# TUMFTM/CamRaDepth

Measured on AMD Instinct MI355X. Metric: training images/sec at 256x416 bf16, higher is better.
Workload: dtype bf16; 1 GPU; CamRaDepth base (image+radar) train step, 8x7x256x416 per GPU, bf16 MFMA / fp32 accumulate, diffGradNorm + OneCycleLR, Dropout2d/DropPath on; global_batch=8, parallelism=dp1, hip_graph=True

## Files before the change

### camradepth_amd/csrc/train_ops.hip

```cpp
#include <math.h>
#include "common.h"

namespace {

constexpr int TPB = 256;

constexpr int OPT_CHUNK = 4096;

template <bool GATED, bool CLIP = false>
__global__ __launch_bounds__(TPB) void k_dgn_norm(const float* p, const float* g, const long long* seg_off, const int* blk2seg,
                                                  const int* blk2chunk, float wd, const float* hp, float* norm_sq,
                                                  const unsigned char* active, int* gate, long long ps = 0) {
  if (hp) wd = hp[3];
  const int t = blk2seg[blockIdx.x];
  if (active && !active[t]) {
    if (threadIdx.x == 0) {
      norm_sq[blockIdx.x] = 0.f;
      if (CLIP) norm_sq[blockIdx.x + ps] = norm_sq[blockIdx.x + 2 * ps] = norm_sq[blockIdx.x + 3 * ps] = 0.f;
    }
    return;
  }
  const long long beg = seg_off[2 * t] + (long long)blk2chunk[blockIdx.x] * OPT_CHUNK;
  long long end = beg + OPT_CHUNK;
  if (end > seg_off[2 * t + 1]) end = seg_off[2 * t + 1];
// ... 191 lines not shown
  const long long tid = (long long)blockIdx.x * TPB + threadIdx.x, stride = (long long)gridDim.x * TPB;
  float4* a4 = reinterpret_cast<float4*>(a + head);
  float4* b4 = reinterpret_cast<float4*>(b + head);
  for (long long i = tid; i < nvec; i += stride) {
    const float4 x = a4[i], y = b4[i];
    a4[i] = y; b4[i] = x;
  }
  const long long tail0 = head + 4 * nvec, rem = head + (n - tail0);
  for (long long i = tid; i < rem; i += stride) {
    const long long j = i < head ? i : tail0 + (i - head);
    const float x = a[j], y = b[j];
    a[j] = y; b[j] = x;
  }
}

constexpr int WP_CO = 16, WP_ELEMS = 512;
__global__ __launch_bounds__(TPB) void k_weight_pack(const crd_pack_entry* tab) {
  __shared__ float tile[WP_CO * WP_ELEMS];
  const crd_pack_entry e = tab[blockIdx.y];
  int ci_t = (WP_ELEMS / e.taps) & ~7;
  if (ci_t < 8) ci_t = 8;
  if (ci_t > 64) ci_t = 64;
  const int n_ci = (e.Cin_pad + ci_t - 1) / ci_t, n_co = (e.Cout_pad + WP_CO - 1) / WP_CO;
  const int per_co = ci_t * e.taps;
  for (int tl = blockIdx.x; tl < n_ci * n_co; tl += gridDim.x) {
    const int co0 = (tl / n_ci) * WP_CO, ci0 = (tl % n_ci) * ci_t;
    __syncthreads();
    for (int i = threadIdx.x; i < WP_CO * per_co; i += TPB) {
      const int co = co0 + i / per_co, r = i % per_co;
      const int ci = ci0 + r / e.taps, tap = r % e.taps;
      float v = 0.f;
      if (co < e.Cout && ci < e.Cin_pad) {
        const int cr = e.cmap ? e.cmap[ci] : (ci < e.Cin_ref ? ci : -1);
        if (cr >= 0) v = e.src[((long long)co * e.Cin_ref + cr) * e.taps + tap];
      }
      tile[i] = v;
    }
    __syncthreads();
    if (e.dst_fwd) {
      for (int i = threadIdx.x; i < WP_CO * per_co; i += TPB) {
        const int cl = i % ci_t, r = i / ci_t;
        const int tap = r % e.taps, col = r / e.taps;
        const int co = co0 + col, ci = ci0 + cl;
        if (co < e.Cout && ci < e.Cin_pad) {
          const float v = tile[col * per_co + cl * e.taps + tap];
          const long long o = ((long long)co * e.taps + tap) * e.Cin_pad + ci;
          if (e.dst_f32) reinterpret_cast<float*>(e.dst_fwd)[o] = e.dst_f32 == 2 ? bf_round(v) : v;
          else reinterpret_cast<bf16_t*>(e.dst_fwd)[o] = f2bf(v);
        }
      }
    }
    if (e.dst_dgrad || e.dst_scatter) {
      for (int i = threadIdx.x; i < WP_CO * per_co; i += TPB) {
        const int col = i % WP_CO, r = i / WP_CO;
        const int tap = r % e.taps, cl = r / e.taps;
        const int co = co0 + col, ci = ci0 + cl;
        if (co < e.Cout_pad && ci < e.Cin_pad) {
          const bf16_t q = f2bf(tile[col * per_co + cl * e.taps + tap]);
          if (e.dst_dgrad) {
            if (e.dgrad_ld == 0) reinterpret_cast<bf16_t*>(e.dst_dgrad)[((long long)ci * e.taps + tap) * e.Cout_pad + co] = q;
            else {
              const int rr = ci - e.dgrad_row0;
              if (rr >= 0 && rr < e.dgrad_rows)
                reinterpret_cast<bf16_t*>(e.dst_dgrad)[((long long)rr * e.taps + tap) * e.dgrad_ld + e.dgrad_coff + co] = q;
            }
          }
          if (e.dst_scatter) reinterpret_cast<bf16_t*>(e.dst_scatter)[((long long)tap * e.Cin_pad + ci) * e.Cout_pad + co] = q;
        }
      }
    }
  }
}

__global__ __launch_bounds__(TPB) void k_wgrad_unpack(const crd_unpack_entry* tab, int accumulate) {
  const crd_unpack_entry e = tab[blockIdx.y];
  const long long n = (long long)e.Cout * e.taps * e.Cin_pad;
  for (long long i = (long long)blockIdx.x * TPB + threadIdx.x; i < n; i += (long long)gridDim.x * TPB) {
    const int ci = (int)(i % e.Cin_pad);
    const long long r = i / e.Cin_pad;
    const int tap = (int)(r % e.taps), co = (int)(r / e.taps);
    const int cr = e.cmap ? e.cmap[ci] : (ci < e.Cin_ref ? ci : -1);
    if (cr < 0) continue;
    float* d = e.dst + ((long long)co * e.Cin_ref + cr) * e.taps + tap;
    float v;
    if (e.src_sum) {
      const crd_sum_t* src = reinterpret_cast<const crd_sum_t*>(e.src);
      long long q = src[i], q1 = 0, q2 = 0, q3 = 0;
      int rp = 1;
      for (; rp + 3 <= e.replicas; rp += 3) {
        q1 += src[(long long)rp * e.replica_stride + i];
        q2 += src[(long long)(rp + 1) * e.replica_stride + i];
        q3 += src[(long long)(rp + 2) * e.replica_stride + i];
      }
      for (; rp < e.replicas; ++rp) q += src[(long long)rp * e.replica_stride + i];
      v = (float)(q + q1 + q2 + q3) * (1.f / GRAD_ONE);
    } else {
      const float* src = reinterpret_cast<const float*>(e.src);
      float v1 = 0.f, v2 = 0.f, v3 = 0.f;
      v = src[i];
      int rp = 1;
      for (; rp + 3 <= e.replicas; rp += 3) {
        v1 += src[(long long)rp * e.replica_stride + i];
        v2 += src[(long long)(rp + 1) * e.replica_stride + i];
        v3 += src[(long long)(rp + 2) * e.replica_stride + i];
      }
      for (; rp < e.replicas; ++rp) v += src[(long long)rp * e.replica_stride + i];
      v += (v1 + v2) + v3;
    }
    *d = accumulate ? *d + v : v;
  }
}

__global__ __launch_bounds__(TPB) void k_dropout_masks(float* out, const float* keep, int rows, int cols, unsigned long long seed,
                                                       unsigned long long* counter) {
  const unsigned long long epoch = *counter;
  const long long total = (long long)rows * cols;
  for (long long i = (long long)blockIdx.x * TPB + threadIdx.x; i < total; i += (long long)gridDim.x * TPB) {
    const int r = (int)(i / cols);
    const float kp = keep[r];
    const unsigned long long h = splitmix64(splitmix64(seed ^ (epoch * 0xD1342543DE82EF95ull)) + (unsigned long long)i);
    const float u = (float)(h >> 40) * (1.0f / 16777216.0f);
    out[i] = u < kp ? 1.0f / kp : 0.0f;
  }
}
__global__ void k_counter_inc(unsigned long long* counter) { *counter += 1; }
// ... 99 lines not shown
  hipLaunchKernelGGL(k_swap_f32, dim3(blocks_for(work, TPB, 4096)), dim3(TPB), 0, as_stream(stream), a, b, (long long)n, head, nvec);
  CRD_LAUNCH_CHECK("crd_swap_f32");
  return CRD_OK;
}

extern "C" int crd_dropout_masks(float* out, const float* keep, int32_t rows, int32_t cols, uint64_t seed, uint64_t* counter,
                                 crd_stream_t stream) {
  CRD_CHECK_ARG(out && keep && counter && rows > 0 && cols > 0, "crd_dropout_masks: bad argument");
  hipLaunchKernelGGL(k_dropout_masks, dim3(blocks_for((long long)rows * cols, TPB, 64)), dim3(TPB), 0, as_stream(stream), out, keep, rows,
                     cols, (unsigned long long)seed, reinterpret_cast<unsigned long long*>(counter));
  hipLaunchKernelGGL(k_counter_inc, dim3(1), dim3(1), 0, as_stream(stream), reinterpret_cast<unsigned long long*>(counter));
  CRD_LAUNCH_CHECK("crd_dropout_masks");
  return CRD_OK;
}

extern "C" int crd_weight_pack(const crd_pack_entry* table_dev, int32_t n, int64_t max_elems, crd_stream_t stream) {
  CRD_CHECK_ARG(table_dev && n > 0 && max_elems > 0, "crd_weight_pack: bad argument");
  long long tiles = (max_elems + WP_CO * WP_ELEMS - 1) / (WP_CO * WP_ELEMS) * 2;
  if (tiles < 1) tiles = 1;
  if (tiles > 96) tiles = 96;
  hipLaunchKernelGGL(k_weight_pack, dim3((unsigned)tiles, n), dim3(TPB), 0, as_stream(stream), table_dev);
  CRD_LAUNCH_CHECK("crd_weight_pack");
  return CRD_OK;
}

extern "C" int crd_wgrad_unpack(const crd_unpack_entry* table_dev, int32_t n, int64_t max_elems, int32_t accumulate,
                                crd_stream_t stream) {
  CRD_CHECK_ARG(table_dev && n > 0 && max_elems > 0, "crd_wgrad_unpack: bad argument");
  hipLaunchKernelGGL(k_wgrad_unpack, dim3(blocks_for(max_elems, TPB, 2048), n), dim3(TPB), 0, as_stream(stream), table_dev, accumulate);
  CRD_LAUNCH_CHECK("crd_wgrad_unpack");
  return CRD_OK;
}
```

### camradepth_amd/engine.py

```python
import bisect
import os
from types import SimpleNamespace as Rec

import torch

from . import lib as L
from . import trace
from . import plan_tables as tables
from . import plan_values
from .config import MID_CHANNELS, UNSUP_CLASSES
from .plan_desc import make_desc
from .plan_values import (BF16, F32, SUM, PM, ConvW, Op, _BufPtr, _Lazy, _WPtr, conv3p_tile, dgrad_flops, fp8_tile,
                          fused_reduce_tile_ok, gn_small_tile, gnbwd_tile, gngemm_tile, halo_tile, igemm_tile, nbytes,
                          persistent_conv3, rup, wgrad3_tile, wgrad_tile)

_DEV = os.environ.get("CRD_DEV_SWITCHES") == "1"


def _dev_flag(name):
    return _DEV and os.environ.get(name) is not None


def _dev_int(name, default):
    return int(os.environ.get(name, default)) if _DEV else int(default)
# ... 1 lines not shown

FUSE_GN_RED_MAXPIX = _dev_int("CRD_FUSE_GN_RED_MAXPIX", 416)


def gn_conv_default():
    return _dev_int("CRD_GN_CONV", 2)


MLP_FUSED = _dev_int("CRD_MLP_FUSED", 1) != 0
MLP_FUSED_MAXPIX = _dev_int("CRD_MLP_FUSED_MAXPIX", 128)
FC2_FOLD_MINROWS = _dev_int("CRD_FC2_FOLD_MINROWS", 16384)
GN_CONV_MAXROWS = _dev_int("CRD_GN_CONV_MAXROWS", 1 << 30)
W3_LATE_WGS = _dev_int("CRD_W3_LATE_WGS", 160)
LATE = 3
DW_REPLICAS = tables.DW_REPLICAS
HEAD_ROWS = 64
GNB_FC1 = _dev_int("CRD_GNB_FC1", 7)
GNB_SR = _dev_int("CRD_GNB_SR", 15)
QSR_GROUP = _dev_int("CRD_QSR_GROUP", 4)


class Plan:
    def __init__(self, model, B, H, W, training):
        cfg = model.cfg
        assert H % 32 == 0 and W % 32 == 0, "H and W must be multiples of 32 (SURVEY.md section 8 note on 900x1600)"
        self.model, self.cfg, self.B, self.H, self.W, self.training = model, cfg, B, H, W, training
        self.dev = model.flat.device
        self.lib = L.load()
        self.fwd, self.bwd_groups, self.bwd_tags = [], [], []
        self._tag = "enc0"
# ... 959 lines not shown
        bad = ~torch.isfinite(self.model.flat_grad)
        if not bool(bad.any()) and bool(torch.isfinite(self.zb_arena).all()):
            return
        where = int(bad.nonzero()[0]) if bool(bad.any()) else -1
        pname = "zb_arena"
        for n_, o_ in zip(self.model._names, self.model._offsets):
            if o_ <= where:
                pname = n_
        for k in self.keep:
            if isinstance(k, tuple) and k[0] == "buf" and k[5].is_floating_point() and not bool(torch.isfinite(k[5].float()).all()):
                print("[crd] non-finite buffer", k[1:5], flush=True)
        raise L.CrdError(f"non-finite gradient after op {i} {op.name} (first bad param {pname})")

    def _unpack(self, tag, stream):
        if tag in self.unpack_ranges:
            lo, hi, mx = self.unpack_ranges[tag]
            L.check(self.lib.crd_wgrad_unpack(self.unpack_table.data_ptr() + lo * self.unpack_stride, hi - lo, mx, 1, stream),
                    "crd_wgrad_unpack")

    def pack(self, lo=None, hi=None):
        st = L.stream()
        i0 = 0 if lo is None else bisect.bisect_left(self.pack_offs, lo)
        i1 = self.n_pack if hi is None else bisect.bisect_left(self.pack_offs, hi)
        if i1 > i0:
            L.check(self.lib.crd_weight_pack(self.pack_table.data_ptr() + i0 * self.pack_stride, i1 - i0,
                                             max(self.pack_elems[i0:i1]), st), "crd_weight_pack")
        base = self.model.flat.data_ptr()
        for cw, cin16 in self.fp8_convs:
            off = (self.p(cw.name + ".weight").data_ptr() - base) // 4
            if (lo is None or off >= lo) and (hi is None or off < hi):
                L.check(self.lib.crd_weight_quant_fp8(cw.w_fwd.data_ptr(), cw.cout, 9, cw.cin_pad, cin16, cw.w8.data_ptr(),
                                                      cw.w8_scales.data_ptr(), st), "crd_weight_quant_fp8")
        for cw, Wt, rows, K, W8, W8s in self.fp8_kcat:
            off = (self.p(cw.name + ".weight").data_ptr() - base) // 4
            if (lo is None or off >= lo) and (hi is None or off < hi):
                L.check(self.lib.crd_weight_quant_fp8(Wt.data_ptr(), rows, 9, K, K, W8.data_ptr(), W8s.data_ptr(), st), "crd_weight_quant_fp8")
        if lo is None and hi is None:
            self.packed_version = getattr(self.model, "_param_version", 0)

    def ensure_packed(self):
        if self.packed_version != getattr(self.model, "_param_version", 0):
# ... 43 lines not shown
```

### camradepth_amd/lib.py

```python
import ctypes as C
import os
import struct

import torch

_HERE = os.path.dirname(os.path.abspath(__file__))
LIB_PATH = os.environ.get("CRD_LIB") or os.path.join(_HERE, "libcamradepth_hip.so")


class CrdError(RuntimeError):
    pass


class ConvDesc(C.Structure):
    _fields_ = [
        ("x", C.c_void_p), ("x_ld", C.c_int32), ("x_coff", C.c_int32),
        ("B", C.c_int32), ("IH", C.c_int32), ("IW", C.c_int32), ("Cin", C.c_int32),
        ("w", C.c_void_p), ("Cout", C.c_int32), ("KH", C.c_int32), ("KW", C.c_int32),
        ("stride", C.c_int32), ("pad", C.c_int32), ("OH", C.c_int32), ("OW", C.c_int32),
        ("gather_mode", C.c_int32),
        ("y", C.c_void_p), ("y_ld", C.c_int32), ("y_coff", C.c_int32), ("y_f32", C.c_int32),
        ("out_mode", C.c_int32), ("patch_k", C.c_int32), ("patch_c", C.c_int32),
        ("bias", C.c_void_p), ("bias_bstride", C.c_int32), ("act", C.c_int32),
        ("res", C.c_void_p), ("res_ld", C.c_int32), ("res_scale", C.c_void_p),
# ... 42 lines not shown


class MlpDesc(C.Structure):
    _fields_ = [(n, C.c_void_p) for n in ("x1", "x1_stats", "norm_gamma", "norm_beta", "w_fc1", "b_fc1", "norm1_gamma", "norm1_beta",
                                          "w9", "b_dw", "norm2_gamma", "norm2_beta", "w_fc2", "xn", "h1", "h2", "h3", "h1_stats",
                                          "h2_stats", "fc2_partials")] + \
               [(n, C.c_int32) for n in ("B", "H", "W", "C", "hidden")]


class UnpackEntry(C.Structure):
    _fields_ = [
        ("src", C.c_void_p), ("dst", C.c_void_p), ("cmap", C.c_void_p),
        ("Cout", C.c_int32), ("Cin_ref", C.c_int32), ("taps", C.c_int32), ("Cin_pad", C.c_int32),
        ("replicas", C.c_int32), ("src_sum", C.c_int32), ("replica_stride", C.c_int64),
    ]


class DgnDesc(C.Structure):
    _fields_ = [(n, C.c_void_p) for n in ("p", "g", "exp_avg", "exp_avg_sq", "prev_grad", "exp_grad_norm", "factor", "parts", "seg_off",
                                          "blk2seg", "blk2chunk", "active", "hp_dev", "gate", "clip", "ema")] + \
               [("parts_stride", C.c_int64), ("n_tensors", C.c_int32), ("n_blocks", C.c_int32)] + \
               [(n, C.c_float) for n in ("lr", "beta1", "beta2", "eps", "weight_decay")] + \
               [("step", C.c_int32), ("max_norm", C.c_float), ("ema_decay", C.c_float),
                ("ema_warmup", C.c_int32), ("ema_n", C.c_int32), ("ema_base", C.c_int32)]


_lib = None
ABI_VERSION = 13


# ... 31 lines not shown
    "crd_conv_igemm": "pp", "crd_conv_igemm_route": "ppi", "crd_gn_conv": "ppp", "crd_gn_conv2": "ppppp", "crd_gn_bwd_conv": "ppp", "crd_pw_narrow_supported": "iii", "crd_tune_pw_narrow": "i", "crd_conv3x3_fp8": "ppfp", "crd_amax_bf16": "pliiipp", "crd_quant_fp8": "pliiipiifp",
    "crd_weight_quant_fp8": "piiiippp", "crd_conv3x3_fp8_dgrad": "pppp", "crd_gn_bwd_apply_fp8": "piiipiiiiiipippipppppiipiippp",
    "crd_fp8_scale_update": "ppifip", "crd_quant_fp8_dev": "pliiipiipp", "crd_tune_conv3x3_small_grid": "i", "crd_tune_igemm_reg_epilogue": "i", "crd_conv_wgrad": "pp", "crd_conv_wgrad_splits": "p", "crd_conv_wgrad_route": "ppi", "crd_wgrad_group_build": "piplp", "crd_conv_wgrad_grouped": "ppp",
    "crd_gn_stats": "piiiiiippp", "crd_gn_apply": "piiiiiipippipPiiip".replace("P", "p"),
    "crd_gn_bwd_reduce": "piiipiiiiiipippippplp", "crd_gn_bwd_apply": "piiipiiiiiipippipppppiiiipipp",
    "crd_gn_launch_shape": "iiiippp",
    "crd_dwconv3x3": "piiiippipppippppppp", "crd_dwconv3x3_wgrad": "ppiiiipipippp",
    "crd_attn_scores": "ppiiiiifppp", "crd_attn_scores_fp8": "ppiiiiffppp", "crd_attn_fwd": "ppiiiiifpppppppppp", "crd_attn_xbar": "ppppiiipp", "crd_attn_xbar_proj": "pppppiiippp", "crd_attn_vec_bwd": "ppiiifppp", "crd_attn_out_residual": "pppppiiipp", "crd_attn_out_residual_stats": "pppppiiippp",
    "crd_attn_out_bwd": "ppppiiipppp", "crd_attn_out_bwd_blocks": "iii", "crd_attn_out_bwd_gn": "ppppiiippppppppppp", "crd_attn_scores_bwd": "ppppiiiiifpppp", "crd_attn_bwd": "ppppiiiiifpppppifppp", "crd_attn_scores_bwd_partials": "iiiii", "crd_sum_partials_bf16": "pilplp", "crd_gsum_to_bf16": "pplp",
    "crd_attn_bwd_fused_supported": "iiiii", "crd_attn_bwd_fused": "ppppppp" "iiiii" "f" "ppppp" "ppppppp" "p", "crd_attn_dk_fold": "pilpl" "pp" "iii" "f" "pp" "p",
    "crd_bicubic2x": "piiiiiipiip", "crd_bicubic2x_fp8": "piiiiiipiifpiip", "crd_gn_apply_fp8": "piiiiiipippippiifpiip", "crd_bicubic2x_bwd": "piiiiiipiiip",
    "crd_input_grad": "ppppiiiiiipp",
    "crd_nchw_to_pm": "piiiipiiip", "crd_pm_to_nchw": "piiiiiiipp", "crd_seg_argmax": "piiiiipiiip", "crd_scale_f32": "pplfp",
    "crd_slice_copy": "piipiiliip", "crd_f32_to_bf16_rows": "pipiiliplpiip", "crd_dropout_masks": "ppiiLpp", "crd_sigmoid_bwd": "pplp", "crd_head_conv2_fwd": "pppiiippiip", "crd_head_conv2_bwd": "ppiippiiippip", "crd_head_conv2_bwd_data": "ppiippiiipp", "crd_head_conv2_wgrad": "ppiipiiipip",
    "crd_weight_pack": "pilp", "crd_wgrad_unpack": "pilip",
    "crd_assemble_input": "pppiiifpp", "crd_gt_pyramid": "piiifppppp",
    "crd_augment_draw": "ppiiiiifffffffiLLp", "crd_augment_lut": "piipp", "crd_augment_assemble": "pppppppiiiiifppppp",
    "crd_augment_gather": "ppppiiiiiippppp", "crd_gt_pyramid_from_full": "piiipppp",
    "crd_radar_project": "pppiipppipiiiffpppppppp", "crd_radar_rasterize": "ppppppppiipiiiiiplppp",
    "crd_lidar_project": "pppiippppippipppipiiiffLLpppppppppp", "crd_lidar_ground_truth": "pppppppppiipiiiiipppipLplpppp",
    "crd_depth_unproject": "piiiiipipiiLLLipppppp", "crd_point_cloud": "piiiiipipiiLLLipppipplpppppp",
    "crd_bev_grid": "ppppiiipiLLLiiLLiiiplppppppp",
    "crd_occupancy_update": "pppiiipipipiiiiLiLLLLiiiiiipppppplpppppp",
    "crd_distance_field": "piiiiiippplppppp", "crd_field_paths": "pppiipLpppiiiiiippppppp",
    "crd_nav_field": "piiippipLiiipppp", "crd_nav_paths": "ppiipLppiiipppppp",
    "crd_map_objects": "piiiiiiipLplpppppp",
    "crd_track_objects": "pppp" "iiiii" "LLLL" "ii" "ppppppppp" "p",
    "crd_match_scan": "ppp" "iii" "pipi" "iii" "LLLL" "i" "ppp" "ii" "p" "il" "pl" "ppppppp" "p",
    "crd_plan_rollouts": "pppp" "iiii" "pLpp" "iiii" "ppp" "iii" "LL" "pLL" "iiiii" "pl" "pppp" "ppppp" "p" "p",
    "crd_viz_range": "piiiiipplpp", "crd_viz_draw": "piiiippffipiiffipllp", "crd_seg_labels": "piiiipp",
# ... 44 lines not shown
    if nonfinite(reset=False):
        v = torch.full_like(v, float("nan"))
    return v


def f64_bits(x):
    return struct.unpack("<Q", struct.pack("<d", float(x)))[0]


def check(rc, what=""):
    if rc != 0:
        msg = load().crd_last_error().decode()
        raise CrdError(f"{what} failed with status {rc}: {msg}")


def conv_route(desc):
    buf = C.create_string_buffer(96)
    check(load().crd_conv_igemm_route(C.byref(desc), buf, len(buf)), "crd_conv_igemm_route")
    return buf.value.decode()


def wgrad_route(desc):
    buf = C.create_string_buffer(96)
    check(load().crd_conv_wgrad_route(C.byref(desc), buf, len(buf)), "crd_conv_wgrad_route")
    return buf.value.decode()


def gn_launch_shape(P, Cn, B, kind):
    out = (C.c_int32 * 3)()
    ptr = [C.cast(C.byref(out, 4 * i), C.c_void_p) for i in range(3)]
# ... 11 lines not shown
```

### camradepth_amd/plan_tables.py

```python
import ctypes as C

import torch

from . import lib as L
from .plan_values import BF16, F32, SUM, rup

SEGMENTS = ["dec", "enc3", "enc2", "enc1", "enc0"]
DW_REPLICAS = 16


def _struct_table(entries, dev):
    if not entries:
        return torch.zeros(8, dtype=torch.uint8, device=dev)
    raw = b"".join(bytes(e) for e in entries)
    return torch.frombuffer(bytearray(raw), dtype=torch.uint8).to(dev)


def _pack_entry(plan, name, dims, cmap=None, **dst):
    e = L.PackEntry()
    e.src = plan.p(name + ".weight").data_ptr()
    e.cmap = cmap.data_ptr() if cmap is not None else None
    e.Cout, e.Cin_ref, e.taps, e.Cin_pad, e.Cout_pad = dims
    for k, v in dst.items():
        setattr(e, k, v.data_ptr() if isinstance(v, torch.Tensor) else v)
    return e


def build_pack_table(plan):
    dev = plan.dev
    sizes = lambda cw: (cw.cout * cw.taps * cw.cin_pad, cw.cin_pad * cw.taps * cw.cout_pad)
# ... 18 lines not shown
            cw.cmap_dev = torch.tensor(cw.cmap, dtype=torch.int32, device=dev)
        dst = {k: t for k, t in (("dst_fwd", cw.w_fwd), ("dst_dgrad", cw.w_dgrad), ("dst_scatter", cw.w_scatter)) if t is not None}
        entries.append((_pack_entry(plan, cw.name, cw.dims, cw.cmap_dev, **dst), max(n_fwd, n_bwd)))
    for (cw, Wt, ld, coff, row0, rows) in plan.kcat_entries:
        entries.append((_pack_entry(plan, cw.name, cw.dims, cw.cmap_dev, dst_dgrad=Wt, dgrad_ld=ld, dgrad_coff=coff, dgrad_row0=row0,
                                    dgrad_rows=rows), cw.cin_pad * cw.taps * cw.cout_pad))
    for (name, hid, w9, fmt) in plan.dw_entries:
        entries.append((_pack_entry(plan, name, (1, hid, 9, hid, 8), dst_fwd=w9, dst_f32=fmt), 9 * hid))
    base = plan.model.flat.data_ptr()
    entries.sort(key=lambda en: en[0].src)
    plan.pack_offs = [(e.src - base) // 4 for e, _ in entries]
    plan.pack_elems = [n for _, n in entries]
    plan.pack_table = _struct_table([e for e, _ in entries], dev)
    plan.pack_stride = C.sizeof(L.PackEntry)
    plan.n_pack = len(entries)


def stream3_splits(lib, B, ih, iw, cin, cout, k=3, stride=1, pad=1, wg_budget=0):
    probe = L.WgradDesc()
    probe.B, probe.IH, probe.IW, probe.OH, probe.OW = B, ih, iw, (ih + 2 * pad - k) // stride + 1, (iw + 2 * pad - k) // stride + 1
    probe.Cin, probe.Cout, probe.KH, probe.KW, probe.stride, probe.pad = cin, cout, k, k, stride, pad
    probe.wg_budget = wg_budget
    return int(lib.crd_conv_wgrad_splits(C.byref(probe)))


def place_weight_gradients(plan):
    out = []
    for cw in plan.convs:
        if cw.frozen:
            continue
# ... 38 lines not shown
        items.append((cw.tag, _unpack_entry(dst=plan.g(cw.name + ".weight"), dims=cw.dims[:4], cmap=cw.cmap_dev, **parts), nel))
    for name, hid, dw10, tag in plan.dw_grads:
        for which, taps, row in (("weight", 9, 0), ("bias", 1, 9)):
            items.append((tag, _unpack_entry(dw10.t.data_ptr() + row * hid * 8, plan.g(name + "." + which), (1, hid, taps, hid),
                                             replicas=DW_REPLICAS, replica_stride=10 * hid), taps * hid))
    for name, Cn, rows, R, tag, off, stride in plan.row_grads:
        items.append((tag, _unpack_entry(rows.t.data_ptr() + 8 * off, plan.g(name), (1, Cn, 1, Cn), replicas=R, replica_stride=stride), Cn))
    items.sort(key=lambda it: SEGMENTS.index(it[0]))
    plan.unpack_ranges = {}
    for i, (tag, _, nel) in enumerate(items):
        lo, _, mx = plan.unpack_ranges.get(tag, (i, i, 1))
        plan.unpack_ranges[tag] = (lo, i + 1, max(mx, nel))
    plan.unpack_table = _struct_table([u for _, u, _ in items], plan.dev)
    plan.unpack_stride = C.sizeof(L.UnpackEntry)
    plan.n_unpack, plan.max_unpack = len(items), max([1] + [nel for _, _, nel in items])


def order_backward(plan):
    written = {}
    plan.bwd, plan.bwd_segments = [], []
    for grp, tag in zip(reversed(plan.bwd_groups), reversed(plan.bwd_tags)):
        if plan.bwd_segments and plan.bwd_segments[-1][0] == tag:
            plan.bwd_segments[-1][2] = len(plan.bwd) + len(grp)
        else:
            plan.bwd_segments.append([tag, len(plan.bwd), len(plan.bwd) + len(grp)])
        for op in grp:
            if op.region is not None:
                key, c0, c1 = op.region[:-2], op.region[-2], op.region[-1]
                prev = written.setdefault(key, [])
                overlap = [r for r in prev if r[0] < c1 and c0 < r[1]]
# ... 11 lines not shown
```

### include/camradepth_hip.h

```cpp
#ifndef CAMRADEPTH_HIP_H
#define CAMRADEPTH_HIP_H

#include <stdint.h>

#ifdef __cplusplus
extern "C" {
#endif

typedef void* crd_stream_t;

#define CRD_OK 0
#define CRD_E_INVALID (-1)
#define CRD_E_UNSUPPORTED (-2)
#define CRD_E_LAUNCH (-3)

typedef int64_t crd_sum_t;
#define CRD_STAT_FRAC_BITS 20
#define CRD_GRAD_FRAC_BITS 44
int crd_nonfinite_status(int32_t reset, crd_stream_t stream);
int crd_nonfinite_capture(int32_t* window_flag, crd_stream_t stream);

const char* crd_last_error(void);
#define CRD_ABI_VERSION 13
int crd_version(void);
// ... 235 lines not shown
  int32_t dst_f32;
  int32_t dgrad_ld, dgrad_coff, dgrad_row0, dgrad_rows;
} crd_pack_entry;
int crd_weight_pack(const crd_pack_entry* table_dev, int32_t n, int64_t max_elems, crd_stream_t stream);
typedef struct {
  const void* src;
  float* dst;
  const int32_t* cmap;
  int32_t Cout, Cin_ref, taps, Cin_pad;
  int32_t replicas;
  int32_t src_sum;
  int64_t replica_stride;
} crd_unpack_entry;
int crd_wgrad_unpack(const crd_unpack_entry* table_dev, int32_t n, int64_t max_elems, int32_t accumulate,
                     crd_stream_t stream);

int crd_dropout_masks(float* out, const float* keep, int32_t rows, int32_t cols, uint64_t seed, uint64_t* counter,
                      crd_stream_t stream);

int crd_assemble_input(const void* img_u8, const float* radar, const float* rad_vel, int32_t B, int32_t H, int32_t W,
                       float max_depth, float* out, crd_stream_t stream);
int crd_gt_pyramid(const float* depth, int32_t B, int32_t H, int32_t W, float max_depth, float* full, float* half,
                   float* quarter, float* eighth, crd_stream_t stream);
int crd_resize_nearest_u8(const void* src, int32_t B, int32_t SH, int32_t SW, int32_t C, void* dst, int32_t DH, int32_t DW,
                          crd_stream_t stream);
int crd_resize_labels_nearest(const void* src_u8, int32_t B, int32_t SH, int32_t SW, int32_t rows, int64_t* dst, int32_t DH,
                              int32_t DW, crd_stream_t stream);

#define CRD_AUGMENT_WORDS 8
#define CRD_AUGMENT_STREAM 0xA0761D6478BD642Full
// ... 182 lines not shown
```

Before: 478.2 images/s.

## Tile weight pack/unpack via precomputed work-item lists with larger LDS tiles

Replaces the 2D-grid weight pack and wgrad unpack kernels with tiled versions that use larger shared-memory tiles, padded strides, fast integer division and unrolled gathers. The host precomputes flat work-item lists, so each block handles a balanced tile or a run of small entries instead of launching max_elems-sized grids per entry. The goal is to cut wasted blocks and uncoalesced strided accesses in per-step weight repacking and gradient unpacking. In exchange the host-side planning gets more complex, and the tile-shape heuristics may not suit every layer.

```diff
diff --git a/camradepth_amd/csrc/train_ops.hip b/camradepth_amd/csrc/train_ops.hip
--- a/camradepth_amd/csrc/train_ops.hip
+++ b/camradepth_amd/csrc/train_ops.hip
@@ -229,101 +229,300 @@
   }
 }
 
-constexpr int WP_CO = 16, WP_ELEMS = 512;
-__global__ __launch_bounds__(TPB) void k_weight_pack(const crd_pack_entry* tab) {
-  __shared__ float tile[WP_CO * WP_ELEMS];
+constexpr int WP_LDS = 12288;
+constexpr int UP_LDS = 4608;
+constexpr int PACK_ITEM_WORK = WP_LDS;
+constexpr int UNPACK_ITEM_WORK = UP_LDS;
+constexpr int PACK_MAX_TAPS = 64, UNPACK_MAX_TAPS = 512;
+constexpr int PACK_LOAD_UNR = 16, PACK_UNR = 8, UNPACK_UNR = 4, UNPACK_UNR1 = 8;
+
+struct FastDiv { unsigned m; int one; };
+__host__ __device__ inline FastDiv fast_div(int d) { return FastDiv{d <= 1 ? 0u : 0xFFFFFFFFu / (unsigned)d + 1u, d <= 1 ? 1 : 0}; }
+__device__ __forceinline__ int fdiv(int r, FastDiv f) { return (int)__umulhi((unsigned)r, f.m) + r * f.one; }
+template <typename T>
+__device__ __forceinline__ __attribute__((address_space(1))) T* as_global(T* p) {
+  return (__attribute__((address_space(1))) T*)p;
+}
+__host__ __device__ inline int imin(int a, int b) { return a < b ? a : b; }
+__host__ __device__ inline int imax(int a, int b) { return a > b ? a : b; }
+__host__ __device__ inline int pack_co_ext(const crd_pack_entry& e) { return imax(e.Cout, e.Cout_pad); }
+
+__host__ __device__ inline void pack_shape(const crd_pack_entry& e, int& co_t, int& ci_t) {
+  const int tp = e.taps | 1, cin8 = (e.Cin_pad + 7) & ~7, co_ext = pack_co_ext(e);
+  for (co_t = 64;; co_t >>= 1) {
+    const int per = WP_LDS / imin(co_t, co_ext);
+    ci_t = imin(imin(((per - 1) / tp) & ~7, cin8), 512);
+    if (co_t == 16 || ci_t >= imin(cin8, 16)) break;
+  }
+  if (ci_t < 8) ci_t = 8;
+}
+
+__host__ __device__ inline void unpack_shape(const crd_unpack_entry& e, int& ci_sh, int& rows) {
+  const int tp = e.taps | 1, rep = imax(e.replicas, 1);
+  int sh = 12;
+  while (sh > 3 && (tp << sh) > 4096) --sh;
+  while (sh > 3 && (1 << (sh - 1)) >= e.Cin_pad) --sh;
+  while (sh > 6 && (long long)(e.taps << sh) * rep > UNPACK_ITEM_WORK) --sh;
+  ci_sh = sh;
+  const long long w1 = (long long)e.taps * imin(1 << sh, e.Cin_pad) * rep;
+  rows = imax(1, imin(imin(UP_LDS / (tp << sh), (int)(UNPACK_ITEM_WORK / w1)), e.Cout));
+}
+
+__device__ __forceinline__ int pow2_shift(int n) {
+  int s = 0;
+  while ((1 << s) < n) ++s;
+  return s;
+}
+
+struct PackTile { int co0, ci0, co_n, ci_n, row, taps, tp, pc; FastDiv by_taps; };
+
+template <bool CMAP>
+__device__ __forceinline__ void pack_load(const crd_pack_entry& e, const PackTile& t, float* tile) {
+  const int total = t.co_n * t.row, taps = t.taps;
+  const FastDiv by_row = fast_div(t.row);
+  const auto* src0 = as_global(e.src);
+  const auto* s = src0 + (long long)t.co0 * e.Cin_ref * taps;
+  const auto* cmap = as_global(e.cmap);
+  const int src_row = e.Cin_ref * taps, co_live = e.Cout - t.co0;
+  for (int i0 = threadIdx.x; i0 < total; i0 += TPB * PACK_LOAD_UNR) {
+    int at[PACK_LOAD_UNR], cr[PACK_LOAD_UNR], so[PACK_LOAD_UNR];
+    float v[PACK_LOAD_UNR];
+#pragma unroll
+    for (int u = 0; u < PACK_LOAD_UNR; ++u) {
+      const int idx = i0 + u * TPB, ix = idx < total ? idx : 0;
+      const int col = fdiv(ix, by_row), r = ix - col * t.row;
+      const int cl = fdiv(r, t.by_taps), tap = r - cl * taps, ci = t.ci0 + cl;
+      at[u] = idx < total ? col * t.pc + cl * t.tp + tap : -1;
+      so[u] = col < co_live ? col * src_row + tap : -1;
+      cr[u] = CMAP ? cmap[ci] : (ci < e.Cin_ref ? ci : -1);
+    }
+#pragma unroll
+    for (int u = 0; u < PACK_LOAD_UNR; ++u) {
+      if (so[u] < 0) cr[u] = -1;
+      v[u] = *(cr[u] >= 0 ? s + (so[u] + cr[u] * taps) : src0);
+    }
+#pragma unroll
+    for (int u = 0; u < PACK_LOAD_UNR; ++u)
+      if (at[u] >= 0) tile[at[u]] = cr[u] >= 0 ? v[u] : 0.f;
+  }
+}
+
+__device__ void pack_tile(const crd_pack_entry& e, int co0, int ci0, int co_t, int ci_t, float* tile) {
+  PackTile t;
+  t.co0 = co0, t.ci0 = ci0, t.taps = e.taps, t.tp = e.taps | 1, t.pc = (ci_t * t.tp) | 1;
+  t.co_n = imin(co_t, pack_co_ext(e) - co0), t.ci_n = imin(ci_t, e.Cin_pad - ci0);
+  t.row = t.ci_n * t.taps;
+  t.by_taps = fast_div(t.taps);
+  const int taps = t.taps, tp = t.tp, pc = t.pc, co_n = t.co_n, ci_n = t.ci_n, row = t.row;
+  const int tid = threadIdx.x;
+  __syncthreads();
+  if (e.cmap) pack_load<true>(e, t, tile);
+  else pack_load<false>(e, t, tile);
+  __syncthreads();
+  if (e.dst_fwd) {
+    const int gsh = pow2_shift(ci_n), g1 = (1 << gsh) - 1;
+    const int rows_n = imin(co_n, e.Cout - co0) * taps;
+    const long long base = (long long)co0 * taps * e.Cin_pad + ci0;
+    auto* d32 = as_global(reinterpret_cast<float*>(e.dst_fwd)) + base;
+    auto* d16 = as_global(reinterpret_cast<bf16_t*>(e.dst_fwd)) + base;
+#pragma unroll 4
+    for (int idx = tid; idx < (rows_n << gsh); idx += TPB) {
+      const int cl = idx & g1, q = idx >> gsh;
+      if (cl < ci_n) {
+        const int col = fdiv(q, t.by_taps), tap = q - col * taps;
+        const float v = tile[col * pc + cl * tp + tap];
+        const int o = q * e.Cin_pad + cl;
+        if (e.dst_f32) d32[o] = e.dst_f32 == 2 ? bf_round(v) : v;
+        else d16[o] = f2bf(v);
+      }
+    }
+  }
+  if (e.dst_dgrad || e.dst_scatter) {
+    const int cp_n = imin(co_n, e.Cout_pad - co0);
+    const int gsh = pow2_shift(cp_n), g1 = (1 << gsh) - 1;
+    auto* dg = as_global(reinterpret_cast<bf16_t*>(e.dst_dgrad));
+    auto* sc = as_global(reinterpret_cast<bf16_t*>(e.dst_scatter));
+    if (dg && e.dgrad_ld == 0) dg += (long long)ci0 * taps * e.Cout_pad + co0;
+#pragma unroll 4
+    for (int idx = tid; idx < (row << gsh); idx += TPB) {
+      const int col = idx & g1, r = idx >> gsh;
+      if (col < cp_n) {
+        const int cl = fdiv(r, t.by_taps), tap = r - cl * taps;
+        const bf16_t q = f2bf(tile[col * pc + cl * tp + tap]);
+        const int ci = ci0 + cl, co = co0 + col;
+        if (dg) {
+          if (e.dgrad_ld == 0) dg[r * e.Cout_pad + col] = q;
+          else {
+            const int rr = ci - e.dgrad_row0;
+            if (rr >= 0 && rr < e.dgrad_rows) dg[(long long)(rr * taps + tap) * e.dgrad_ld + e.dgrad_coff + co] = q;
+          }
+        }
+        if (sc) sc[(long long)(tap * e.Cin_pad + ci) * e.Cout_pad + co] = q;
+      }
+    }
+  }
+}
+
+__global__ __launch_bounds__(TPB) void k_weight_pack(const crd_pack_entry* tab, const crd_work_item* items) {
+  __shared__ float tile[WP_LDS];
+  const crd_work_item it = items[blockIdx.x];
+  for (int k = 0; k < it.n_entries; ++k) {
+    const crd_pack_entry e = tab[it.entry + k];
+    int co_t, ci_t;
+    pack_shape(e, co_t, ci_t);
+    pack_tile(e, it.co0, it.ci0, co_t, ci_t, tile);
+  }
+}
+
+__global__ __launch_bounds__(TPB) void k_weight_pack_grid(const crd_pack_entry* tab) {
+  __shared__ float tile[WP_LDS];
   const crd_pack_entry e = tab[blockIdx.y];
-  int ci_t = (WP_ELEMS / e.taps) & ~7;
-  if (ci_t < 8) ci_t = 8;
-  if (ci_t > 64) ci_t = 64;
-  const int n_ci = (e.Cin_pad + ci_t - 1) / ci_t, n_co = (e.Cout_pad + WP_CO - 1) / WP_CO;
-  const int per_co = ci_t * e.taps;
-  for (int tl = blockIdx.x; tl < n_ci * n_co; tl += gridDim.x) {
-    const int co0 = (tl / n_ci) * WP_CO, ci0 = (tl % n_ci) * ci_t;
-    __syncthreads();
-    for (int i = threadIdx.x; i < WP_CO * per_co; i += TPB) {
-      const int co = co0 + i / per_co, r = i % per_co;
-      const int ci = ci0 + r / e.taps, tap = r % e.taps;
-      float v = 0.f;
-      if (co < e.Cout && ci < e.Cin_pad) {
-        const int cr = e.cmap ? e.cmap[ci] : (ci < e.Cin_ref ? ci : -1);
-        if (cr >= 0) v = e.src[((long long)co * e.Cin_ref + cr) * e.taps + tap];
+  int co_t, ci_t;
+  pack_shape(e, co_t, ci_t);
+  const int n_ci = (e.Cin_pad + ci_t - 1) / ci_t, n_co = (pack_co_ext(e) + co_t - 1) / co_t;
+  for (int tl = blockIdx.x; tl < n_ci * n_co; tl += gridDim.x) pack_tile(e, (tl / n_ci) * co_t, (tl % n_ci) * ci_t, co_t, ci_t, tile);
+}
+
+template <int N, typename P, typename A>
+__device__ __forceinline__ void unpack_fold(P src, const int (&i)[N], int replicas, long long stride, A (&out)[N]) {
+  A v1[N], v2[N], v3[N];
+#pragma unroll
+  for (int u = 0; u < N; ++u) {
+    out[u] = src[i[u]];
+    v1[u] = v2[u] = v3[u] = 0;
+  }
+  int rp = 1;
+  P p = src + stride;
+  for (; rp + 3 <= replicas; rp += 3, p += 3 * stride) {
+    A a[N], b[N], c[N];
+#pragma unroll
+    for (int u = 0; u < N; ++u) {
+      a[u] = p[i[u]];
+      b[u] = p[stride + i[u]];
+      c[u] = p[2 * stride + i[u]];
+    }
+#pragma unroll
+    for (int u = 0; u < N; ++u) {
+      v1[u] += a[u];
+      v2[u] += b[u];
+      v3[u] += c[u];
+    }
+  }
+  for (; rp < replicas; ++rp, p += stride) {
+#pragma unroll
+    for (int u = 0; u < N; ++u) out[u] += p[i[u]];
+  }
+#pragma unroll
+  for (int u = 0; u < N; ++u) out[u] += (v1[u] + v2[u]) + v3[u];
+}
+
+struct UnpackTile { int co0, ci0, sh, ci_m, ci_n, taps, tp, per, total; FastDiv by_taps; };
+
+template <bool CMAP>
+__device__ __forceinline__ void unpack_store(const crd_unpack_entry& e, const UnpackTile& t, int accumulate, const float* lds) {
+  auto* dst = as_global(e.dst) + (long long)t.co0 * e.Cin_ref * t.taps;
+  const auto* cmap = as_global(e.cmap);
+  for (int i0 = threadIdx.x; i0 < t.total; i0 += TPB * PACK_UNR) {
+    int o[PACK_UNR], cm[PACK_UNR];
+    float v[PACK_UNR], old[PACK_UNR];
+#pragma unroll
+    for (int u = 0; u < PACK_UNR; ++u) {
+      const int idx = i0 + u * TPB;
+      const int x = fdiv(idx, t.by_taps), tap = idx - x * t.taps;
+      const int col = x >> t.sh, cl = x & t.ci_m;
+      const bool ok = idx < t.total && cl < t.ci_n;
+      const int cx = ok ? t.ci0 + cl : t.ci0;
+      cm[u] = CMAP ? cmap[cx] : (cx < e.Cin_ref ? cx : -1);
+      o[u] = ok ? col * e.Cin_ref * t.taps + tap : -1;
+      v[u] = lds[ok ? col * t.per + cl * t.tp + tap : 0];
+    }
+#pragma unroll
+    for (int u = 0; u < PACK_UNR; ++u) o[u] = o[u] >= 0 && cm[u] >= 0 ? o[u] + cm[u] * t.taps : -1;
+    if (accumulate) {
+#pragma unroll
+      for (int u = 0; u < PACK_UNR; ++u) old[u] = dst[o[u] >= 0 ? o[u] : 0];
+#pragma unroll
+      for (int u = 0; u < PACK_UNR; ++u) v[u] = old[u] + v[u];
+    }
+#pragma unroll
+    for (int u = 0; u < PACK_UNR; ++u)
+      if (o[u] >= 0) dst[o[u]] = v[u];
+  }
+}
+
+template <int N, bool FOLD, bool SUM>
+__device__ __forceinline__ void unpack_gather(const crd_unpack_entry& e, const UnpackTile& t, float* lds) {
+  const long long base = (long long)t.co0 * t.taps * e.Cin_pad + t.ci0;
+  for (int i0 = threadIdx.x; i0 < t.total; i0 += TPB * N) {
+    int i[N], at[N];
+    float v[N];
+#pragma unroll
+    for (int u = 0; u < N; ++u) {
+      const int idx = i0 + u * TPB, cl = idx & t.ci_m, q = idx >> t.sh;
+      const bool ok = idx < t.total && cl < t.ci_n;
+      const int col = fdiv(q, t.by_taps), tap = q - col * t.taps;
+      i[u] = ok ? q * e.Cin_pad + cl : 0;
+      at[u] = ok ? col * t.per + cl * t.tp + tap : -1;
+    }
+    if (SUM) {
+      long long s[N];
+      const auto* src = as_global(reinterpret_cast<const crd_sum_t*>(e.src)) + base;
+      if (FOLD) unpack_fold<N>(src, i, e.replicas, (long long)e.replica_stride, s);
+      else {
+#pragma unroll
+        for (int u = 0; u < N; ++u) s[u] = src[i[u]];
       }
-      tile[i] = v;
-    }
-    __syncthreads();
-    if (e.dst_fwd) {
-      for (int i = threadIdx.x; i < WP_CO * per_co; i += TPB) {
-        const int cl = i % ci_t, r = i / ci_t;
-        const int tap = r % e.taps, col = r / e.taps;
-        const int co = co0 + col, ci = ci0 + cl;
-        if (co < e.Cout && ci < e.Cin_pad) {
-          const float v = tile[col * per_co + cl * e.taps + tap];
-          const long long o = ((long long)co * e.taps + tap) * e.Cin_pad + ci;
-          if (e.dst_f32) reinterpret_cast<float*>(e.dst_fwd)[o] = e.dst_f32 == 2 ? bf_round(v) : v;
-          else reinterpret_cast<bf16_t*>(e.dst_fwd)[o] = f2bf(v);
-        }
+#pragma unroll
+      for (int u = 0; u < N; ++u) v[u] = (float)s[u] * (1.f / GRAD_ONE);
+    } else {
+      const auto* src = as_global(reinterpret_cast<const float*>(e.src)) + base;
+      if (FOLD) unpack_fold<N>(src, i, e.replicas, (long long)e.replica_stride, v);
+      else {
+#pragma unroll
+        for (int u = 0; u < N; ++u) v[u] = src[i[u]];
       }
     }
-    if (e.dst_dgrad || e.dst_scatter) {
-      for (int i = threadIdx.x; i < WP_CO * per_co; i += TPB) {
-        const int col = i % WP_CO, r = i / WP_CO;
-        const int tap = r % e.taps, cl = r / e.taps;
-        const int co = co0 + col, ci = ci0 + cl;
-        if (co < e.Cout_pad && ci < e.Cin_pad) {
-          const bf16_t q = f2bf(tile[col * per_co + cl * e.taps + tap]);
-          if (e.dst_dgrad) {
-            if (e.dgrad_ld == 0) reinterpret_cast<bf16_t*>(e.dst_dgrad)[((long long)ci * e.taps + tap) * e.Cout_pad + co] = q;
-            else {
-              const int rr = ci - e.dgrad_row0;
-              if (rr >= 0 && rr < e.dgrad_rows)
-                reinterpret_cast<bf16_t*>(e.dst_dgrad)[((long long)rr * e.taps + tap) * e.dgrad_ld + e.dgrad_coff + co] = q;
-            }
-          }
-          if (e.dst_scatter) reinterpret_cast<bf16_t*>(e.dst_scatter)[((long long)tap * e.Cin_pad + ci) * e.Cout_pad + co] = q;
-        }
-      }
-    }
-  }
-}
-
-__global__ __launch_bounds__(TPB) void k_wgrad_unpack(const crd_unpack_entry* tab, int accumulate) {
+#pragma unroll
+    for (int u = 0; u < N; ++u)
+      if (at[u] >= 0) lds[at[u]] = v[u];
+  }
+}
+
+__device__ void unpack_tile(const crd_unpack_entry& e, int co0, int ci0, int sh, int rows, int accumulate, float* lds) {
+  UnpackTile t;
+  t.co0 = co0, t.ci0 = ci0, t.sh = sh, t.ci_m = (1 << sh) - 1, t.taps = e.taps, t.tp = e.taps | 1, t.per = t.tp << sh;
+  t.ci_n = imin(1 << sh, e.Cin_pad - ci0);
+  t.total = (imin(rows, e.Cout - co0) * t.taps) << sh;
+  t.by_taps = fast_div(t.taps);
+  __syncthreads();
+  if (e.replicas <= 1) {
+    if (e.src_sum) unpack_gather<UNPACK_UNR1, false, true>(e, t, lds);
+    else unpack_gather<UNPACK_UNR1, false, false>(e, t, lds);
+  } else if (e.src_sum) unpack_gather<UNPACK_UNR / 2, true, true>(e, t, lds);
+  else unpack_gather<UNPACK_UNR, true, false>(e, t, lds);
+  __syncthreads();
+  if (e.cmap) unpack_store<true>(e, t, accumulate, lds);
+  else unpack_store<false>(e, t, accumulate, lds);
+}
+
+__global__ __launch_bounds__(TPB) void k_wgrad_unpack(const crd_unpack_entry* tab, const crd_work_item* items, int accumulate) {
+  __shared__ float lds[UP_LDS];
+  const crd_work_item it = items[blockIdx.x];
+  for (int k = 0; k < it.n_entries; ++k) {
+    const crd_unpack_entry e = tab[it.entry + k];
+    int sh, rows;
+    unpack_shape(e, sh, rows);
+    unpack_tile(e, it.co0, it.ci0, sh, rows, accumulate, lds);
+  }
+}
+
+__global__ __launch_bounds__(TPB) void k_wgrad_unpack_grid(const crd_unpack_entry* tab, int accumulate) {
+  __shared__ float lds[UP_LDS];
   const crd_unpack_entry e = tab[blockIdx.y];
-  const long long n = (long long)e.Cout * e.taps * e.Cin_pad;
-  for (long long i = (long long)blockIdx.x * TPB + threadIdx.x; i < n; i += (long long)gridDim.x * TPB) {
-    const int ci = (int)(i % e.Cin_pad);
-    const long long r = i / e.Cin_pad;
-    const int tap = (int)(r % e.taps), co = (int)(r / e.taps);
-    const int cr = e.cmap ? e.cmap[ci] : (ci < e.Cin_ref ? ci : -1);
-    if (cr < 0) continue;
-    float* d = e.dst + ((long long)co * e.Cin_ref + cr) * e.taps + tap;
-    float v;
-    if (e.src_sum) {
-      const crd_sum_t* src = reinterpret_cast<const crd_sum_t*>(e.src);
-      long long q = src[i], q1 = 0, q2 = 0, q3 = 0;
-      int rp = 1;
-      for (; rp + 3 <= e.replicas; rp += 3) {
-        q1 += src[(long long)rp * e.replica_stride + i];
-        q2 += src[(long long)(rp + 1) * e.replica_stride + i];
-        q3 += src[(long long)(rp + 2) * e.replica_stride + i];
-      }
-      for (; rp < e.replicas; ++rp) q += src[(long long)rp * e.replica_stride + i];
-      v = (float)(q + q1 + q2 + q3) * (1.f / GRAD_ONE);
-    } else {
-      const float* src = reinterpret_cast<const float*>(e.src);
-      float v1 = 0.f, v2 = 0.f, v3 = 0.f;
-      v = src[i];
-      int rp = 1;
-      for (; rp + 3 <= e.replicas; rp += 3) {
-        v1 += src[(long long)rp * e.replica_stride + i];
-        v2 += src[(long long)(rp + 1) * e.replica_stride + i];
-        v3 += src[(long long)(rp + 2) * e.replica_stride + i];
-      }
-      for (; rp < e.replicas; ++rp) v += src[(long long)rp * e.replica_stride + i];
-      v += (v1 + v2) + v3;
-    }
-    *d = accumulate ? *d + v : v;
-  }
+  int sh, rows;
+  unpack_shape(e, sh, rows);
+  const int n_ci = (e.Cin_pad + (1 << sh) - 1) >> sh, n_co = (e.Cout + rows - 1) / rows;
+  for (int tl = blockIdx.x; tl < n_ci * n_co; tl += gridDim.x) unpack_tile(e, (tl / n_ci) * rows, (tl % n_ci) << sh, sh, rows, accumulate, lds);
 }
 
 __global__ __launch_bounds__(TPB) void k_dropout_masks(float* out, const float* keep, int rows, int cols, unsigned long long seed,
@@ -453,12 +652,112 @@
   return CRD_OK;
 }
 
+namespace {
+constexpr int WORK_RUN_ENTRIES = 4;
+struct WorkTiles { int co_n, co_step, ci_n, ci_step, taps, rep; };
+struct WorkListWriter {
+  crd_work_item* out;
+  int64_t n = 0, max_work = 0, total = 0;
+  int g_entry = 0, g_n = 0;
+  int64_t g_work = 0;
+  void emit(int entry, int n_entries, int co0, int ci0, int64_t work) {
+    if (out) out[n] = crd_work_item{entry, n_entries, co0, ci0};
+    ++n;
+    total += work;
+    if (work > max_work) max_work = work;
+  }
+  void flush() {
+    if (g_n) emit(g_entry, g_n, 0, 0, g_work);
+    g_n = 0;
+    g_work = 0;
+  }
+  void add(int entry, const WorkTiles& t, int64_t item_work) {
+    const int64_t per = (int64_t)t.taps * t.rep, whole = per * t.co_n * t.ci_n;
+    if (t.co_n <= t.co_step && t.ci_n <= t.ci_step && 2 * whole <= item_work) {
+      if (g_n && (g_work + whole > item_work || g_n == WORK_RUN_ENTRIES)) flush();
+      if (!g_n) g_entry = entry;
+      ++g_n;
+      g_work += whole;
+      return;
+    }
+    flush();
+    for (int co0 = 0; co0 < t.co_n; co0 += t.co_step)
+      for (int ci0 = 0; ci0 < t.ci_n; ci0 += t.ci_step)
+        emit(entry, 1, co0, ci0, per * imin(t.co_step, t.co_n - co0) * imin(t.ci_step, t.ci_n - ci0));
+  }
+};
+}
+
+extern "C" int crd_work_items_build(int32_t kind, const void* host_table, int32_t n, const int32_t* bounds, int32_t n_ranges,
+                                    crd_work_item* host_items, int64_t capacity, int32_t* range_items, crd_work_info* info) {
+  CRD_CHECK_ARG((kind == CRD_WORK_PACK || kind == CRD_WORK_UNPACK) && host_table && n > 0 && bounds && n_ranges > 0 && info,
+                "crd_work_items_build: bad argument (kind, a null table, bounds or info, n <= 0 or n_ranges <= 0)");
+  CRD_CHECK_ARG(bounds[0] == 0 && bounds[n_ranges] == n, "crd_work_items_build: bad argument (bounds must run from 0 to n)");
+  for (int r = 0; r < n_ranges; ++r)
+    CRD_CHECK_ARG(bounds[r] <= bounds[r + 1], "crd_work_items_build: bad argument (bounds[%d] > bounds[%d])", r, r + 1);
+  const crd_pack_entry* pk = static_cast<const crd_pack_entry*>(host_table);
+  const crd_unpack_entry* up = static_cast<const crd_unpack_entry*>(host_table);
+  for (int i = 0; i < n; ++i) {
+    const int co = kind == CRD_WORK_PACK ? pk[i].Cout : up[i].Cout, ci = kind == CRD_WORK_PACK ? pk[i].Cin_pad : up[i].Cin_pad;
+    const int taps = kind == CRD_WORK_PACK ? pk[i].taps : up[i].taps;
+    CRD_CHECK_ARG(co > 0 && ci > 0 && taps > 0, "crd_work_items_build: bad argument (entry %d: Cout, Cin_pad or taps <= 0)", i);
+    CRD_UNSUPPORTED(taps <= (kind == CRD_WORK_PACK ? PACK_MAX_TAPS : UNPACK_MAX_TAPS), "crd_work_items_build: entry %d has %d taps", i,
+                        taps);
+  }
+  const int64_t item_work = kind == CRD_WORK_PACK ? PACK_ITEM_WORK : UNPACK_ITEM_WORK;
+  for (int pass = host_items ? 0 : 1; pass < 2; ++pass) {
+    WorkListWriter w{pass == 0 ? nullptr : host_items};
+    for (int r = 0; r < n_ranges; ++r) {
+      if (range_items && (pass == 1)) range_items[r] = (int32_t)w.n;
+      for (int i = bounds[r]; i < bounds[r + 1]; ++i) {
+        WorkTiles t;
+        if (kind == CRD_WORK_PACK) {
+          int co_t, ci_t;
+          pack_shape(pk[i], co_t, ci_t);
+          t = WorkTiles{pack_co_ext(pk[i]), co_t, pk[i].Cin_pad, ci_t, pk[i].taps, 1};
+        } else {
+          int sh, rows;
+          unpack_shape(up[i], sh, rows);
+          t = WorkTiles{up[i].Cout, rows, up[i].Cin_pad, 1 << sh, up[i].taps, imax(up[i].replicas, 1)};
+        }
+        w.add(i, t, item_work);
+      }
+      w.flush();
+    }
+    if (pass == 0) {
+      CRD_CHECK_ARG(capacity >= w.n * (int64_t)sizeof(crd_work_item), "crd_work_items_build: the list needs %lld bytes, capacity is %lld",
+                    (long long)(w.n * (int64_t)sizeof(crd_work_item)), (long long)capacity);
+      continue;
+    }
+    if (range_items) range_items[n_ranges] = (int32_t)w.n;
+    info->n_items = (int32_t)w.n;
+    info->item_work = (int32_t)item_work;
+    info->bytes = w.n * (int64_t)sizeof(crd_work_item);
+    info->max_work = w.max_work;
+    info->total_work = w.total;
+  }
+  return CRD_OK;
+}
+
+extern "C" int crd_weight_pack_items(const crd_pack_entry* table_dev, const crd_work_item* items_dev, int32_t n_items,
+                                     crd_stream_t stream) {
+  CRD_CHECK_ARG(table_dev && items_dev && n_items > 0, "crd_weight_pack_items: bad argument");
+  hipLaunchKernelGGL(k_weight_pack, dim3(n_items), dim3(TPB), 0, as_stream(stream), table_dev, items_dev);
+  CRD_LAUNCH_CHECK("crd_weight_pack_items");
+  return CRD_OK;
+}
+
+extern "C" int crd_wgrad_unpack_items(const crd_unpack_entry* table_dev, const crd_work_item* items_dev, int32_t n_items,
+                                      int32_t accumulate, crd_stream_t stream) {
+  CRD_CHECK_ARG(table_dev && items_dev && n_items > 0, "crd_wgrad_unpack_items: bad argument");
+  hipLaunchKernelGGL(k_wgrad_unpack, dim3(n_items), dim3(TPB), 0, as_stream(stream), table_dev, items_dev, accumulate);
+  CRD_LAUNCH_CHECK("crd_wgrad_unpack_items");
+  return CRD_OK;
+}
+
 extern "C" int crd_weight_pack(const crd_pack_entry* table_dev, int32_t n, int64_t max_elems, crd_stream_t stream) {
   CRD_CHECK_ARG(table_dev && n > 0 && max_elems > 0, "crd_weight_pack: bad argument");
-  long long tiles = (max_elems + WP_CO * WP_ELEMS - 1) / (WP_CO * WP_ELEMS) * 2;
-  if (tiles < 1) tiles = 1;
-  if (tiles > 96) tiles = 96;
-  hipLaunchKernelGGL(k_weight_pack, dim3((unsigned)tiles, n), dim3(TPB), 0, as_stream(stream), table_dev);
+  hipLaunchKernelGGL(k_weight_pack_grid, dim3(blocks_for(max_elems, WP_LDS / 2, 256), n), dim3(TPB), 0, as_stream(stream), table_dev);
   CRD_LAUNCH_CHECK("crd_weight_pack");
   return CRD_OK;
 }
@@ -466,7 +765,8 @@
 extern "C" int crd_wgrad_unpack(const crd_unpack_entry* table_dev, int32_t n, int64_t max_elems, int32_t accumulate,
                                 crd_stream_t stream) {
   CRD_CHECK_ARG(table_dev && n > 0 && max_elems > 0, "crd_wgrad_unpack: bad argument");
-  hipLaunchKernelGGL(k_wgrad_unpack, dim3(blocks_for(max_elems, TPB, 2048), n), dim3(TPB), 0, as_stream(stream), table_dev, accumulate);
+  hipLaunchKernelGGL(k_wgrad_unpack_grid, dim3(blocks_for(max_elems, UP_LDS / 2, 512), n), dim3(TPB), 0, as_stream(stream), table_dev,
+                     accumulate);
   CRD_LAUNCH_CHECK("crd_wgrad_unpack");
   return CRD_OK;
 }
diff --git a/camradepth_amd/engine.py b/camradepth_amd/engine.py
--- a/camradepth_amd/engine.py
+++ b/camradepth_amd/engine.py
@@ -39,6 +39,7 @@
 W3_LATE_WGS = _dev_int("CRD_W3_LATE_WGS", 160)
 LATE = 3
 DW_REPLICAS = tables.DW_REPLICAS
+ITEM_BYTES = 16
 HEAD_ROWS = 64
 GNB_FC1 = _dev_int("CRD_GNB_FC1", 7)
 GNB_SR = _dev_int("CRD_GNB_SR", 15)
@@ -1028,17 +1029,18 @@
 
     def _unpack(self, tag, stream):
         if tag in self.unpack_ranges:
-            lo, hi, mx = self.unpack_ranges[tag]
-            L.check(self.lib.crd_wgrad_unpack(self.unpack_table.data_ptr() + lo * self.unpack_stride, hi - lo, mx, 1, stream),
-                    "crd_wgrad_unpack")
+            lo, hi = self.unpack_item_ranges[tag]
+            L.check(self.lib.crd_wgrad_unpack_items(self.unpack_table.data_ptr(), self.unpack_items.data_ptr() + lo * ITEM_BYTES, hi - lo,
+                                                    1, stream), "crd_wgrad_unpack_items")
 
     def pack(self, lo=None, hi=None):
         st = L.stream()
         i0 = 0 if lo is None else bisect.bisect_left(self.pack_offs, lo)
         i1 = self.n_pack if hi is None else bisect.bisect_left(self.pack_offs, hi)
         if i1 > i0:
-            L.check(self.lib.crd_weight_pack(self.pack_table.data_ptr() + i0 * self.pack_stride, i1 - i0,
-                                             max(self.pack_elems[i0:i1]), st), "crd_weight_pack")
+            lo_it, hi_it = self.pack_item0[i0], self.pack_item0[i1]
+            L.check(self.lib.crd_weight_pack_items(self.pack_table.data_ptr(), self.pack_items.data_ptr() + lo_it * ITEM_BYTES,
+                                                   hi_it - lo_it, st), "crd_weight_pack_items")
         base = self.model.flat.data_ptr()
         for cw, cin16 in self.fp8_convs:
             off = (self.p(cw.name + ".weight").data_ptr() - base) // 4
diff --git a/camradepth_amd/lib.py b/camradepth_amd/lib.py
--- a/camradepth_amd/lib.py
+++ b/camradepth_amd/lib.py
@@ -80,6 +80,17 @@
         ("Cout", C.c_int32), ("Cin_ref", C.c_int32), ("taps", C.c_int32), ("Cin_pad", C.c_int32),
         ("replicas", C.c_int32), ("src_sum", C.c_int32), ("replica_stride", C.c_int64),
     ]
+
+
+class WorkItem(C.Structure):
+    _fields_ = [("entry", C.c_int32), ("n_entries", C.c_int32), ("co0", C.c_int32), ("ci0", C.c_int32)]
+
+
+class WorkInfo(C.Structure):
+    _fields_ = [("n_items", C.c_int32), ("item_work", C.c_int32), ("bytes", C.c_int64), ("max_work", C.c_int64), ("total_work", C.c_int64)]
+
+
+WORK_PACK, WORK_UNPACK = 0, 1
 
 
 class DgnDesc(C.Structure):
@@ -141,6 +152,7 @@
     "crd_nchw_to_pm": "piiiipiiip", "crd_pm_to_nchw": "piiiiiiipp", "crd_seg_argmax": "piiiiipiiip", "crd_scale_f32": "pplfp",
     "crd_slice_copy": "piipiiliip", "crd_f32_to_bf16_rows": "pipiiliplpiip", "crd_dropout_masks": "ppiiLpp", "crd_sigmoid_bwd": "pplp", "crd_head_conv2_fwd": "pppiiippiip", "crd_head_conv2_bwd": "ppiippiiippip", "crd_head_conv2_bwd_data": "ppiippiiipp", "crd_head_conv2_wgrad": "ppiipiiipip",
     "crd_weight_pack": "pilp", "crd_wgrad_unpack": "pilip",
+    "crd_work_items_build": "ipipiplpp", "crd_weight_pack_items": "ppip", "crd_wgrad_unpack_items": "ppiip",
     "crd_assemble_input": "pppiiifpp", "crd_gt_pyramid": "piiifppppp",
     "crd_augment_draw": "ppiiiiifffffffiLLp", "crd_augment_lut": "piipp", "crd_augment_assemble": "pppppppiiiiifppppp",
     "crd_augment_gather": "ppppiiiiiippppp", "crd_gt_pyramid_from_full": "piiipppp",
@@ -215,6 +227,21 @@
         raise CrdError(f"{what} failed with status {rc}: {msg}")
 
 
+def work_items(kind, table_bytes, n, bounds):
+    lib = load()
+    tab = C.create_string_buffer(bytes(table_bytes), len(table_bytes))
+    nr = len(bounds) - 1
+    bnd = (C.c_int32 * (nr + 1))(*bounds)
+    info = WorkInfo()
+    check(lib.crd_work_items_build(kind, C.addressof(tab), n, C.addressof(bnd), nr, None, 0, None, C.addressof(info)),
+          "crd_work_items_build (size)")
+    items = C.create_string_buffer(max(int(info.bytes), 1))
+    ranges = (C.c_int32 * (nr + 1))()
+    check(lib.crd_work_items_build(kind, C.addressof(tab), n, C.addressof(bnd), nr, C.addressof(items), info.bytes, C.addressof(ranges),
+                                   C.addressof(info)), "crd_work_items_build")
+    return items.raw[:info.bytes], list(ranges), info
+
+
 def conv_route(desc):
     buf = C.create_string_buffer(96)
     check(load().crd_conv_igemm_route(C.byref(desc), buf, len(buf)), "crd_conv_igemm_route")
diff --git a/camradepth_amd/plan_tables.py b/camradepth_amd/plan_tables.py
--- a/camradepth_amd/plan_tables.py
+++ b/camradepth_amd/plan_tables.py
@@ -14,6 +14,13 @@
         return torch.zeros(8, dtype=torch.uint8, device=dev)
     raw = b"".join(bytes(e) for e in entries)
     return torch.frombuffer(bytearray(raw), dtype=torch.uint8).to(dev)
+
+
+def _work_list(kind, entries, bounds, dev):
+    if not entries:
+        return torch.zeros(16, dtype=torch.uint8, device=dev), [0] * len(bounds)
+    raw, ranges, _ = L.work_items(kind, b"".join(bytes(e) for e in entries), len(entries), bounds)
+    return torch.frombuffer(bytearray(raw), dtype=torch.uint8).to(dev), ranges
 
 
 def _pack_entry(plan, name, dims, cmap=None, **dst):
@@ -62,6 +69,7 @@
     plan.pack_table = _struct_table([e for e, _ in entries], dev)
     plan.pack_stride = C.sizeof(L.PackEntry)
     plan.n_pack = len(entries)
+    plan.pack_items, plan.pack_item0 = _work_list(L.WORK_PACK, [e for e, _ in entries], list(range(len(entries) + 1)), dev)
 
 
 def stream3_splits(lib, B, ih, iw, cin, cout, k=3, stride=1, pad=1, wg_budget=0):
@@ -130,6 +138,10 @@
     plan.unpack_table = _struct_table([u for _, u, _ in items], plan.dev)
     plan.unpack_stride = C.sizeof(L.UnpackEntry)
     plan.n_unpack, plan.max_unpack = len(items), max([1] + [nel for _, _, nel in items])
+    tags = sorted(plan.unpack_ranges, key=lambda t: plan.unpack_ranges[t][0])
+    bounds = [plan.unpack_ranges[t][0] for t in tags] + [len(items)]
+    plan.unpack_items, ranges = _work_list(L.WORK_UNPACK, [u for _, u, _ in items], bounds, plan.dev)
+    plan.unpack_item_ranges = {t: (ranges[i], ranges[i + 1]) for i, t in enumerate(tags)}
 
 
 def order_backward(plan):
diff --git a/include/camradepth_hip.h b/include/camradepth_hip.h
--- a/include/camradepth_hip.h
+++ b/include/camradepth_hip.h
@@ -273,6 +273,23 @@
 } crd_unpack_entry;
 int crd_wgrad_unpack(const crd_unpack_entry* table_dev, int32_t n, int64_t max_elems, int32_t accumulate,
                      crd_stream_t stream);
+#define CRD_WORK_PACK 0
+#define CRD_WORK_UNPACK 1
+typedef struct crd_work_item {
+  int32_t entry, n_entries, co0, ci0;
+} crd_work_item;
+typedef struct crd_work_info {
+  int32_t n_items;
+  int32_t item_work;
+  int64_t bytes;
+  int64_t max_work;
+  int64_t total_work;
+} crd_work_info;
+int crd_work_items_build(int32_t kind, const void* host_table, int32_t n, const int32_t* bounds, int32_t n_ranges,
+                         crd_work_item* host_items, int64_t capacity, int32_t* range_items, crd_work_info* info);
+int crd_weight_pack_items(const crd_pack_entry* table_dev, const crd_work_item* items_dev, int32_t n_items, crd_stream_t stream);
+int crd_wgrad_unpack_items(const crd_unpack_entry* table_dev, const crd_work_item* items_dev, int32_t n_items, int32_t accumulate,
+                           crd_stream_t stream);
 
 int crd_dropout_masks(float* out, const float* keep, int32_t rows, int32_t cols, uint64_t seed, uint64_t* counter,
                       crd_stream_t stream);
```

Measured after the change: 481.4 images/s (median of 6 runs). No clear change (+0.7%).
